# ericbill21/map-dit

Hardware: AMD Instinct MI355X
Metric: latent-images/sec training step, DiT-B/2 bf16 @256 (higher is better)
Workload: dtype bf16; 1 GPU; DiT-B/2 full training step on 32x32x4 latents (fresh batch+fwd+loss+bwd+grad reduction+Adam+2xEMA), all magnitude-preserving features on, bf16 GEMM operands / fp32 accumulate, master and residual fp32; global_batch=256, per_gpu_batch=256, parallelism=dp1, grad_comm=allreduce-fp32-per-stage-overlapped

## Files before the change

include/mapdit.h:

```cpp
#ifndef MAPDIT_H
#define MAPDIT_H

#include <stddef.h>
#include <stdint.h>

#ifdef __cplusplus
extern "C" {
#endif

#define MAPDIT_OK 0
#define MAPDIT_ERR_ARG 1
#define MAPDIT_ERR_HIP 2

const char* mapdit_last_error(void);
int mapdit_abi_version(void);

enum { MAPDIT_NT = 0, MAPDIT_NN = 1, MAPDIT_TN = 2 };

enum {
    MAPDIT_EPI_STORE_BF16 = 0,
    MAPDIT_EPI_STORE_F32 = 1,
    MAPDIT_EPI_SILU2 = 2,
    MAPDIT_EPI_RESID = 3,
    MAPDIT_EPI_DSILU = 4,
    MAPDIT_EPI_SILU2_COND = 5,
    MAPDIT_EPI_SILU2_GRAD = 7,
    MAPDIT_EPI_MUL_AUX = 8,
    MAPDIT_EPI_RMB = 9,
    MAPDIT_EPI_QKV_HEADS = 6,
    MAPDIT_EPI_QKV_HEADS_RAW = 10
};

typedef struct {
    int kind;
    void* out;
    int ldo;
    void* out2;
    const void* aux;
    const float* gate;
    int ldg;
    int rows_per_sample;
    float alpha, beta;
    int accumulate;
    void* out3;
    const float* shift2;
    const float* scale2;
    const float* gain2;
    int ld2;
    int split_k;
    long slab_stride;
    void* out4;
    const void* rmb;
    int rot2;
} mapdit_epilogue_t;

int mapdit_gemm_bf16(int layout, int M, int N, int K, const uint16_t* A, int lda, const uint16_t* B, int ldb,
                     const mapdit_epilogue_t* epi, void* stream);
typedef struct {
    const uint16_t* A; int lda;
    const uint16_t* B; int ldb;
    int M, N;
    float* out; int ldo;
    float alpha;
    long slab_stride;
} mapdit_gemm_group_item_t;
int mapdit_gemm_group_tn_bf16(int n, const mapdit_gemm_group_item_t* items, int K, int split_k, void* stream);
int mapdit_gemm_tile_size(int M, int N);
int mapdit_gemm_tile_size_ex(int M, int N, int split_k_launch);
int mapdit_gemm_tile_size_k(int M, int N, int K, int split_k_launch);
void mapdit_gemm_tuning(int tile, int phases, long band);

enum { MAPDIT_WN_PLAIN = 2 };
int mapdit_weightnorm_fwd(float* W, int rows, int cols, int forced, float out_scale, uint16_t* w_bf16, float* w_f32,
                          float* inv, void* stream);
typedef struct {
    float* W;
    int rows, cols;
    float out_scale;
    int first_block;
    uint16_t* w_bf16;
    float* w_f32;
    uint16_t* w_split3;
    int flags;
} mapdit_wn_job_t;
int mapdit_weightnorm_fwd_batch(const mapdit_wn_job_t* jobs_dev, int njobs, int total_blocks, int forced, void* stream);
int mapdit_weightnorm_bwd(const float* W, float* G, int ldg, int nslabs, long slab_stride, float* dW, int rows,
                          int cols, float out_scale, int accumulate, void* stream);
int mapdit_weightnorm_bwd_batch(const mapdit_wn_job_t* jobs_dev, int njobs, int total_blocks, void* stream);
typedef struct {
    const float* W; float* G; int ldg; int nslabs; long slab_stride; float* dW; int rows, cols; float out_scale; int flags;
} mapdit_wn_bwd_item_t;
int mapdit_weightnorm_bwd_group(int n, const mapdit_wn_bwd_item_t* items, void* stream);
int mapdit_weightnorm_bwd_slim(const float* W, float* G, int ldg, int nslabs, long slab_stride, float* dW, int rows,
                               int cols, float out_scale, int accumulate, void* stream);

typedef struct {
    long lo, hi, first_block;
} mapdit_range_t;

int mapdit_adam_ema_step(float* params, const float* grads, float* exp_avg, float* exp_avg_sq, float* ema_a,
                         float* ema_b, long n, const float* hyper, float beta1, float beta2, float eps, void* stream);
typedef struct {
    float step_size;
    float inv_sqrt_bc2;
    float ema_beta_a, ema_beta_b;
    float grad_scale;
} mapdit_adam_scalars_t;
int mapdit_adam_ema_step_scalars(float* params, const float* grads, float* exp_avg, float* exp_avg_sq, float* ema_a,
                                 float* ema_b, long n, const mapdit_adam_scalars_t* hyper, float beta1, float beta2,
                                 float eps, void* stream);
int mapdit_grad_nonfinite_check(const float* grads, long n, int* status, int step, void* stream);
int mapdit_adam_ema_step_guarded(float* params, const float* grads, float* exp_avg, float* exp_avg_sq, float* ema_a, float* ema_b,
                                 long n, const mapdit_adam_scalars_t* hyper, float beta1, float beta2, float eps,
                                 const int* status, int step, void* stream);
int mapdit_adam_ema_step_ranges(float* params, const float* grads, float* exp_avg, float* exp_avg_sq, float* ema_a, float* ema_b,
                                const mapdit_range_t* ranges_dev, int nranges, long total_blocks, const mapdit_adam_scalars_t* hyper,
                                float beta1, float beta2, float eps, const int* status, int step, void* stream);
int mapdit_grad_nonfinite_check_ranges(const float* grads, const mapdit_range_t* ranges_dev, int nranges, long total_blocks, int* status,
                                       int step, void* stream);

int mapdit_modulate_fwd(const float* x, const float* shift, const float* scale, int ldmod, const float* gain,
                        uint16_t* out, int n_samples, int T, int D, void* stream);

// ... 255 lines not shown
```

map-dit_amd/_lib.py:

```python
from __future__ import annotations

import ctypes as C
import os
import subprocess
import threading

_HERE = os.path.dirname(os.path.abspath(__file__))
LIB_PATH = os.environ.get("MAPDIT_LIB") or os.path.join(_HERE, "libmapdit_hip.so")
CSRC = os.path.join(_HERE, "csrc")

vp, ci, cf, cl = C.c_void_p, C.c_int, C.c_float, C.c_long


class MapditError(RuntimeError):
    pass


class Epilogue(C.Structure):
    _fields_ = [("kind", ci), ("out", vp), ("ldo", ci), ("out2", vp), ("aux", vp), ("gate", vp), ("ldg", ci),
                ("rows_per_sample", ci), ("alpha", cf), ("beta", cf), ("accumulate", ci), ("out3", vp), ("shift2", vp), ("scale2", vp),
                ("gain2", vp), ("ld2", ci), ("split_k", ci), ("slab_stride", cl), ("out4", vp), ("rmb", vp), ("rot2", ci)]


class ResidModBwd(C.Structure):
# ... 95 lines not shown
    "mapdit_fourier_fwd": [vp, vp, vp, vp, ci, ci, vp],
    "mapdit_cond_combine_fwd": [vp, vp, vp, vp, vp, vp, ci, ci, ci, vp],
    "mapdit_cond_combine_bwd": [vp, vp, vp, vp, vp, vp, ci, ci, ci, vp],
    "mapdit_device_error_poll": [vp],
    "mapdit_comm_unique_id": [vp],
    "mapdit_comm_create": [vp, ci, ci, C.POINTER(vp)],
    "mapdit_allreduce_bucket": [vp, vp, cl, vp],
    "mapdit_reduce_scatter_bucket": [vp, vp, cl, vp],
    "mapdit_allgather_bucket": [vp, vp, cl, vp],
    "mapdit_final_out_fwd": [vp, ci, vp, vp, vp, vp, vp, ci, ci, ci, ci, vp],
    "mapdit_final_out_bwd": [vp, vp, ci, vp, vp, vp, vp, vp, ci, vp, vp, vp, vp, cf, ci, ci, ci, ci, vp],
    "mapdit_cfg_combine": [vp, vp, ci, ci, ci, cf, vp],
    "mapdit_q_sample": [vp, vp, vp, vp, ci, vp, ci, ci, vp],
    "mapdit_loss_fwd": [vp, vp, vp, vp, vp, vp, ci, vp, vp, vp, vp, ci, ci, vp],
    "mapdit_loss_bwd": [vp, vp, vp, vp, vp, ci, ci, vp],
    "mapdit_psample_step": [vp, vp, vp, vp, vp, ci, ci, vp, vp, ci, ci, vp],
    "mapdit_ddim_step": [vp, vp, vp, vp, vp, vp, ci, ci, cf, ci, vp, vp, ci, ci, vp],
    "mapdit_obj_loss_fwd": [vp, vp, vp, vp, vp, vp, vp, ci, ci, ci, ci, vp, vp, vp, vp, ci, ci, vp],
    "mapdit_obj_loss_bwd": [vp, vp, vp, vp, vp, ci, ci, ci, vp],
    "mapdit_obj_step": [vp, vp, vp, vp, vp, vp, ci, ci, ci, ci, ci, cf, vp, vp, ci, ci, vp],
    "mapdit_obj_vb_terms": [vp, vp, vp, vp, vp, vp, vp, ci, ci, ci, ci, vp, vp, vp, vp, ci, ci, ci, ci, vp],
    "mapdit_prior_bpd": [vp, vp, vp, ci, vp, vp, vp, ci, ci, vp],
    "mapdit_engine_create": [C.POINTER(Config), ci, vp, C.c_size_t, vp, C.POINTER(vp)],
    "mapdit_engine_bind": [vp, C.POINTER(vp), C.POINTER(vp)],
    "mapdit_engine_prepare_weights": [vp, ci, vp],
    "mapdit_engine_forward": [vp, vp, vp, vp, ci, ci, vp, vp],
    "mapdit_engine_backward": [vp, vp, vp],
    "mapdit_engine_backward_stages": [vp, vp, ci, ci, vp],
    "mapdit_engine_set_shard": [vp, ci, ci],
    "mapdit_engine_set_block_fences": [vp, C.POINTER(vp), ci],
    "mapdit_engine_weight_image": [vp, ci, C.POINTER(vp), C.POINTER(vp), C.POINTER(ci), C.POINTER(ci), C.POINTER(ci)],
    "mapdit_engine_jacobian_shard": [vp, vp],
    "mapdit_engine_set_loss_scale": [vp, cf],
    "mapdit_engine_loss_scale": [vp, C.POINTER(cf)],
    "mapdit_engine_profile_begin": [vp, ci, ci],
    "mapdit_engine_profile_begin_strided": [vp, ci, ci, ci],
    "mapdit_engine_profile_end": [vp, C.POINTER(ci), C.POINTER(C.c_double)],
    "mapdit_engine_peek": [vp, ci, ci, C.POINTER(vp), C.POINTER(C.c_long), C.POINTER(ci), C.POINTER(ci)],
}
for _n in ("weightnorm_fwd", "weightnorm_fwd_batch", "modulate_fwd", "resid_mod_bwd", "rot_modulate_fwd", "qkv_split",
           "qkv_merge_bwd", "attn_cos_fwd", "attn_cos_fwd_rawqk", "attn_cos_fwd_rawqk_save", "qk_cos_normalize", "attn_cos_bwd", "attn_cos_bwd_fused", "attn_sdpa_fwd", "heads_merge_bwd", "ln_modulate_fwd", "ln_bwd_merge", "qkv_split_generic", "qkv_merge_bwd_generic",
           "attn_generic_fwd", "attn_generic_bwd", "patch_embed_fwd", "cond_combine_fwd", "cond_combine_bwd", "final_out_bwd"):
    _SIGS[f"mapdit_{_n}_f16"] = _SIGS[f"mapdit_{_n}"]
for _b, _h in (("gemm_bf16", "gemm_f16"), ("gemm_group_tn_bf16", "gemm_group_tn_f16"), ("f32_to_bf16", "f32_to_f16"), ("f32_to_bf16_2d", "f32_to_f16_2d"),
               ("mpsilu_to_bf16", "mpsilu_to_f16")):
    _SIGS[f"mapdit_{_h}"] = _SIGS[f"mapdit_{_b}"]
_OTHER = {
    "mapdit_last_error": (C.c_char_p, []),
    "mapdit_abi_version": (ci, []),
    "mapdit_gemm_tile_size": (ci, [ci, ci]),
    "mapdit_gemm_tile_size_ex": (ci, [ci, ci, ci]),
    "mapdit_gemm_tile_size_k": (ci, [ci, ci, ci, ci]),
    "mapdit_gemm_tuning": (None, [ci, ci, cl]),
    "mapdit_engine_workspace_bytes": (C.c_size_t, [C.POINTER(Config), ci]),
    "mapdit_engine_destroy": (None, [vp]),
    "mapdit_comm_destroy": (None, [vp]),
}
EXPORTS = sorted(list(_SIGS) + list(_OTHER))

_lock = threading.Lock()
_handle = None


def _source_digest() -> str:
    import hashlib
    h = hashlib.sha256()
    inc = os.path.join(os.path.dirname(_HERE), "include", "mapdit.h")
    files = sorted(os.path.join(CSRC, f) for f in os.listdir(CSRC) if f.endswith((".hip", ".h")) or f == "Makefile") + [inc]
    for f in files:
        h.update(os.path.basename(f).encode() + b"\0")
        with open(f, "rb") as fh:
            h.update(fh.read())
    return h.hexdigest()


def build(force: bool = False) -> str:
    stamp = LIB_PATH + ".src-sha256"
    digest = _source_digest()
    if not force and os.path.exists(LIB_PATH) and os.path.exists(stamp) and open(stamp).read().strip() == digest:
        return LIB_PATH
    if force:
        subprocess.check_call(["make", "-C", CSRC, "clean"])
    subprocess.check_call(["make", "-C", CSRC, "-j8"])
    with open(stamp, "w") as f:
        f.write(digest + "\n")
    return LIB_PATH


class _Lib:
    def __init__(self, cdll):
        self._cdll = cdll
        for name, argtypes in _SIGS.items():
            fn = getattr(cdll, name)
            fn.argtypes = argtypes
            fn.restype = ci
            setattr(self, name[len("mapdit_"):], self._wrap(name, fn))
        for name, (res, argtypes) in _OTHER.items():
            fn = getattr(cdll, name)
            fn.argtypes = argtypes
            fn.restype = res
            setattr(self, name[len("mapdit_"):], fn)

    def _wrap(self, name, fn):
        def call(*args):
            rc = fn(*args)
            if rc != 0:
# ... 25 lines not shown
```

map-dit_amd/csrc/gemm.hip:

```cpp
#include <stdarg.h>
#include <type_traits>
#include <stdio.h>

#include "common.h"

MD_NS_OPEN

constexpr int BM = 128, BN = 128, BKT = 64;
constexpr int TILE_BYTES = 16384;
constexpr int BUF_BYTES = 2 * TILE_BYTES;
constexpr int CS_LD = 132;
constexpr int SMEM_BYTES = BM * CS_LD * 4;

enum { OP_ROW = 0, OP_KMAJ = 1 };

struct GemmP {
    const bf16_t* A;
    const bf16_t* B;
    int lda, ldb;
    int M, N, K;
    int tiles_n;
    int tiles;
    int split_k;
    int band;
// ... 607 lines not shown
#pragma unroll
        for (int ks = 0; ks < 2; ++ks) {
            bf16x8_t fa[4], fb[2];
#pragma unroll
            for (int i = 0; i < 4; ++i) fa[i] = read_frag<OP_ROW>(cur, i * 16, ks, lane);
#pragma unroll
            for (int j = 0; j < 2; ++j) fb[j] = read_frag<BK>(cur + TILE_BYTES, wave * 32 + j * 16, ks, lane);
            if (BK == OP_KMAJ) {
                asm volatile("s_waitcnt lgkmcnt(0)" ::: "memory");
                __builtin_amdgcn_sched_barrier(0);
            }
#pragma unroll
            for (int i = 0; i < 4; ++i)
#pragma unroll
                for (int j = 0; j < 2; ++j) acc[i][j] = MFMA16(fb[j], fa[i], acc[i][j]);
        }
    }
    __syncthreads();
    float* cs = (float*)smem;
#pragma unroll
    for (int i = 0; i < 4; ++i)
#pragma unroll
        for (int j = 0; j < 2; ++j) {
            const int m = i * 16 + (lane & 15);
            const int n = wave * 32 + j * 16 + 4 * (lane >> 4);
            *(f32x4_t*)(cs + m * CS_LD + n) = acc[i][j];
        }
    __syncthreads();
#pragma unroll
    for (int it = 0; it < 4; ++it) {
        const int row = (tid >> 4) + 16 * it, col = (tid & 15) * 8;
        const int gm = m0 + row, gn = n0 + col;
        if (gm < p.M && gn < p.N) {
            float v[8];
            *(f32x4_t*)(v) = *(const f32x4_t*)(cs + row * CS_LD + col);
            *(f32x4_t*)(v + 4) = *(const f32x4_t*)(cs + row * CS_LD + col + 4);
            epi(gm, gn + p.n_off, v, 0);
        }
    }
}

constexpr int BM2 = 256, BN2 = 256;
constexpr int SLOT_BYTES = 16384, KBUF_BYTES = 4 * SLOT_BYTES;
constexpr int OFF_A0 = 0, OFF_A1 = SLOT_BYTES, OFF_B0 = 2 * SLOT_BYTES, OFF_B1 = 3 * SLOT_BYTES;
constexpr int CS2_LD = 260;
constexpr int SMEM2_BYTES = 128 * CS2_LD * 4;
#ifdef MAPDIT_GEMM_STAMPS
constexpr int STAMP_TILES = 12, STAMP_POINTS = 11;
__device__ long long* g_stamps = nullptr;
__device__ long long* g_wg_times = nullptr;
extern "C" __global__ void mapdit_debug_set_wg_times_kernel(long long* p) { g_wg_times = p; }
__device__ int g_stamp_block = -1;
extern "C" __global__ void mapdit_debug_set_stamps_kernel(long long* p, int block) { g_stamps = p; g_stamp_block = block; }
#define G256_STAMP(PT)                                                                              \
    if (stamp_on && t < STAMP_TILES) {                                                              \
        __builtin_amdgcn_sched_barrier(0);                                                          \
        stamp_lds[(wm * STAMP_TILES + t) * STAMP_POINTS + (PT)] = (long long)__builtin_readcyclecounter(); \
        __builtin_amdgcn_sched_barrier(0);                                                          \
    }
#define G256_TSTAMP(IDX)                                                                            \
    if (wave == 0 && (IDX) < 3) {                        \
        __builtin_amdgcn_sched_barrier(0);                                                          \
        kl_[(IDX) % 3] = (long long)__builtin_readcyclecounter();                                       \
        __builtin_amdgcn_sched_barrier(0);                                                          \
    }                                                                                               \
    if (stamp_on && wave == 0) {                                                                    \
        __builtin_amdgcn_sched_barrier(0);                                                          \
        stamp_lds[2 * STAMP_TILES * STAMP_POINTS + (IDX)] = (long long)__builtin_readcyclecounter(); \
        __builtin_amdgcn_sched_barrier(0);                                                          \
    }
#define G256_RSTAMP(IDX)                                                                            \
    if (stamp_on && wave == 0) {                                                                    \
        __builtin_amdgcn_sched_barrier(0);                                                          \
        stamp_lds[2 * STAMP_TILES * STAMP_POINTS + (IDX)] = (long long)__builtin_amdgcn_s_memrealtime(); \
        __builtin_amdgcn_sched_barrier(0);                                                          \
    }
#define G256_STAMPS_OUT()                                                                           \
    if (g_wg_times && wave == 0 && lane == 0) {                                                     \
        long long* r_ = g_wg_times + 4 * (long long)bid;                                     \
        r_[0] = wg_r0; r_[1] = (long long)__builtin_amdgcn_s_memrealtime();                         \
        const long long now_ = (long long)__builtin_readcyclecounter();                             \
        r_[2] = now_ - wg_t0;                                                                       \
                       \
        r_[3] = ((long long)__builtin_amdgcn_s_getreg(((4 - 1) << 11) | (0 << 6) | 20) & 0xff) |    \
                (((kl_[2] - kl_[1]) & 0xffffff) << 8) | (((kl_[1] - wg_t0) & 0xffff) << 32) |       \
                (((now_ - kl_[2]) & 0xffff) << 48);                                                 \
    }                                                                                               \
    if (stamp_on) {                                                                                 \
        for (int i = 0; i < STAMP_TILES * STAMP_POINTS; ++i)                                        \
            g_stamps[wm * STAMP_TILES * STAMP_POINTS + i] = stamp_lds[wm * STAMP_TILES * STAMP_POINTS + i]; \
        if (wave == 0)                                                                              \
            for (int i = 0; i < 8; ++i) g_stamps[2 * STAMP_TILES * STAMP_POINTS + i] = stamp_lds[2 * STAMP_TILES * STAMP_POINTS + i]; \
    }
#else
#define G256_STAMP(PT)
#define G256_TSTAMP(IDX)
#define G256_RSTAMP(IDX)
#define G256_STAMPS_OUT()
#endif

template <int SIDE> __device__ __forceinline__ int half_map(int i, int h) {
    return SIDE == 0 ? ((i >> 6) * 128 + h * 64 + (i & 63)) : ((i >> 5) * 64 + h * 32 + (i & 31));
}

template <int KIND, int SIDE, bool KTAIL>
__device__ __forceinline__ void stage_half(const bf16_t* __restrict__ G, int ld, int idx0, int idx_max, int k0, int kmax, int h,
// ... 435 lines not shown
    __shared__ __attribute__((aligned(16))) char smem[kReduce<Epi> ? SMEM2_BYTES + 3 * 8 * 256 * 4 : SMEM2_BYTES];
#endif
    const int total = p.tiles * p.split_k;
    stagger_start(p);
    for (int v = blockIdx.x; v < total; v += gridDim.x) {
        gemm256_tile<AK, BK, Epi, KTAIL, FE>(p, epi, smem, v, total);
        __syncthreads();
    }
}

constexpr int GROUP_MAX = 4;
struct GroupArgs {
    GemmP p[GROUP_MAX];
    EpiStoreF32 e[GROUP_MAX];
    int first[GROUP_MAX + 1];
    int n;
};
__global__ __launch_bounds__(512, 2) void gemm_mfma256_group_kernel(GroupArgs g) {
#ifdef MAPDIT_GEMM_STAMPS
    __shared__ __attribute__((aligned(16))) char smem[SMEM2_BYTES + (2 * STAMP_TILES * STAMP_POINTS + 8) * 8];
#else
    __shared__ __attribute__((aligned(16))) char smem[SMEM2_BYTES];
#endif
    const int total = g.first[g.n];
    for (int v = blockIdx.x; v < total; v += gridDim.x) {
        int i = 0;
        while (i + 1 < g.n && v >= g.first[i + 1]) ++i;
        gemm256_tile<OP_KMAJ, OP_KMAJ, EpiStoreF32, false, false>(g.p[i], g.e[i], smem, v - g.first[i], g.first[i + 1] - g.first[i]);
        __syncthreads();
    }
}

struct TileCoord { int m0, n0, z, tile, kbeg, nk; };
__device__ __forceinline__ TileCoord tile_coord(const GemmP& p, const int bid, const int nwg) {
    const int xcd = bid & 7, q = nwg >> 3, r = nwg & 7;
    const int wg = (xcd < r ? xcd * (q + 1) : r * (q + 1) + (xcd - r) * q) + (bid >> 3);
    TileCoord c;
    c.z = wg / p.tiles;
    c.tile = wg - c.z * p.tiles;
    const int tiles_m = p.tiles / p.tiles_n;
    const int bsz = tiles_m * p.band;
    const int bidx = c.tile / bsz, rem = c.tile - bidx * bsz;
    const int bw = (bidx + 1) * p.band <= p.tiles_n ? p.band : p.tiles_n - bidx * p.band;
    c.m0 = (rem / bw) * BM2;
    c.n0 = (bidx * p.band + rem % bw) * BN2;
    const int nkt = (p.K + BKT - 1) / BKT, kbase = nkt / p.split_k, krem = nkt % p.split_k;
    c.kbeg = (c.z * kbase + (c.z < krem ? c.z : krem)) * BKT;
    c.nk = kbase + (c.z < krem ? 1 : 0);
    return c;
}

constexpr int WPRIV_BYTES = 4096;
constexpr int SMEM_W_BYTES = 2 * KBUF_BYTES + 8 * WPRIV_BYTES;

template <int AK, int BK, bool KTAIL>
__device__ __forceinline__ void g256_prologue(const GemmP& p, const TileCoord& c, char* smem, int wave, int lane) {
    stage_half<AK, 0, KTAIL>(p.A, p.lda, c.m0, p.M, c.kbeg, p.K, 0, smem + OFF_A0, wave, lane);
    stage_half<BK, 1, KTAIL>(p.B, p.ldb, c.n0, p.N, c.kbeg, p.K, 0, smem + OFF_B0, wave, lane);
    stage_half<BK, 1, KTAIL>(p.B, p.ldb, c.n0, p.N, c.kbeg, p.K, 1, smem + OFF_B1, wave, lane);
    stage_half<AK, 0, KTAIL>(p.A, p.lda, c.m0, p.M, c.kbeg, p.K, 1, smem + OFF_A1, wave, lane);
    if (c.nk > 1) {
        char* b1 = smem + KBUF_BYTES;
        stage_half<AK, 0, KTAIL>(p.A, p.lda, c.m0, p.M, c.kbeg + BKT, p.K, 0, b1 + OFF_A0, wave, lane);
        stage_half<BK, 1, KTAIL>(p.B, p.ldb, c.n0, p.N, c.kbeg + BKT, p.K, 0, b1 + OFF_B0, wave, lane);
        stage_half<BK, 1, KTAIL>(p.B, p.ldb, c.n0, p.N, c.kbeg + BKT, p.K, 1, b1 + OFF_B1, wave, lane);
    }
}

#ifndef MAPDIT_EPI_PD_AUX
#define MAPDIT_EPI_PD_AUX 2
#endif
template <class Epi> constexpr bool kWaveEpilogue = true;
template <class Epi> constexpr bool kWaveEpilogueAnyK = true;
template <> constexpr bool kWaveEpilogue<EpiResid> = false;
template <> constexpr bool kWaveEpilogue<EpiStoreF32> = false;
template <> constexpr bool kWaveEpilogueAnyK<EpiStoreBf16> = false;
template <class Epi> constexpr int kEpiPrefetch = 2;
template <class Epi> constexpr bool kEpiPipeline = true;
template <> constexpr int kEpiPrefetch<EpiResid> = 1;
template <> constexpr int kEpiPrefetch<EpiMulAux> = MAPDIT_EPI_PD_AUX;
template <> constexpr int kEpiPrefetch<EpiDSilu> = MAPDIT_EPI_PD_AUX;
template <> constexpr bool kEpiPipeline<EpiResid> = false;
template <class Epi, bool INTERIOR>
__device__ __forceinline__ void g256w_epilogue(const GemmP& p, const Epi& epi, const TileCoord& c, f32x4_t (&acc)[8][4],
                                               char* priv, const int wave, const int lane) {
    const int wm = wave >> 2, wn = wave & 3;
    const int cch = lane & 7, rsub = lane >> 3;
    const int wrow = lane & 15, wq = lane >> 4;
    const int gn = c.n0 + wn * 64 + cch * 8;
    const bool col_ok = INTERIOR || gn < p.N;
    typename Epi::Tile tctx;
    if (col_ok) tctx = epi.tile_begin(c.m0, (c.m0 + BM2 <= p.M ? c.m0 + BM2 : p.M) - 1, gn);
    f32x4_t* b = (f32x4_t*)priv;
    constexpr int PD = kEpiPrefetch<Epi>;
    constexpr bool PIPE = kEpiPipeline<Epi>;
    typename Epi::Aux aux[8][2];
    const int mw = c.m0 + wm * 128 + rsub;
    auto row_of = [&](int r, int s) { return mw + (r >> 2) * 64 + (r & 3) * 16 + 8 * s; };
    int woff[4], roff[2][2];
#pragma unroll
    for (int j = 0; j < 4; ++j) woff[j] = wrow * 16 + ((4 * j + wq) ^ (wrow & 7));
#pragma unroll
    for (int s = 0; s < 2; ++s) {
        const int rr = rsub + 8 * s;
        roff[s][0] = rr * 16 + ((2 * cch) ^ (rr & 7));
        roff[s][1] = rr * 16 + ((2 * cch + 1) ^ (rr & 7));
    }
#pragma unroll
    for (int r = 0; r < PD; ++r)
#pragma unroll
        for (int s = 0; s < 2; ++s)
            if (INTERIOR || (row_of(r, s) < p.M && col_ok)) aux[r][s] = epi.load(row_of(r, s), gn);
    f32x4_t cur[2][2], nxt[2][2];
    if (PIPE) {
#pragma unroll
        for (int j = 0; j < 4; ++j) b[woff[j]] = acc[0][j];
#pragma unroll
        for (int s = 0; s < 2; ++s) { cur[s][0] = b[roff[s][0]]; cur[s][1] = b[roff[s][1]]; }
    }
#pragma unroll
    for (int r = 0; r < 8; ++r) {
        if (r + PD < 8) {
#pragma unroll
            for (int s = 0; s < 2; ++s)
                if (INTERIOR || (row_of(r + PD, s) < p.M && col_ok)) aux[r + PD][s] = epi.load(row_of(r + PD, s), gn);
        }
        if (PIPE && r + 1 < 8) {
#pragma unroll
            for (int j = 0; j < 4; ++j) b[woff[j]] = acc[r + 1][j];
#pragma unroll
            for (int s = 0; s < 2; ++s) { nxt[s][0] = b[roff[s][0]]; nxt[s][1] = b[roff[s][1]]; }
        }
        if (!PIPE) {
#pragma unroll
            for (int j = 0; j < 4; ++j) b[woff[j]] = acc[r][j];
#pragma unroll
            for (int s = 0; s < 2; ++s) { cur[s][0] = b[roff[s][0]]; cur[s][1] = b[roff[s][1]]; }
        }
#pragma unroll
        for (int s = 0; s < 2; ++s) {
            float v[8];
            *(f32x4_t*)(v) = cur[s][0];
            *(f32x4_t*)(v + 4) = cur[s][1];
            if (INTERIOR || (row_of(r, s) < p.M && col_ok)) epi.apply(row_of(r, s), gn, v, c.z, aux[r][s], tctx);
        }
        if (PIPE) {
#pragma unroll
            for (int s = 0; s < 2; ++s) { cur[s][0] = nxt[s][0]; cur[s][1] = nxt[s][1]; }
        }
    }
}

template <int AK, int BK, class Epi, bool KTAIL = false>
__global__ __launch_bounds__(512, 2) void gemm_mfma256w_kernel(GemmP p, Epi epi) {
    __shared__ __attribute__((aligned(16))) char smem[SMEM_W_BYTES];
    const int total = p.tiles * p.split_k;
    int v = blockIdx.x;
    if (v >= total) return;
    stagger_start(p);
    constexpr bool TR_ASM2 = AK == OP_KMAJ;
    TileCoord c = tile_coord(p, v, total);
    {
        const int tid0 = threadIdx.x;
        g256_prologue<AK, BK, KTAIL>(p, c, smem, __builtin_amdgcn_readfirstlane(tid0 >> 6), tid0 & 63);
    }
    bool first = true;
#ifdef MAPDIT_GEMM_STAMPS
    long long ph_[4] = {0, 0, 0, 0};
    int ph_tiles_ = 0;
#define GW_STAMP(VAR) __builtin_amdgcn_sched_barrier(0); const long long VAR = (long long)__builtin_readcyclecounter(); __builtin_amdgcn_sched_barrier(0)
#else
#define GW_STAMP(VAR)
#endif
    for (;;) {
        int tid_ = threadIdx.x;
        asm volatile("" : "+v"(tid_));
        const int tid = tid_, lane = tid & 63;
        const int wave = __builtin_amdgcn_readfirstlane(tid >> 6);
        const int wm = wave >> 2, wn = wave & 3;
        const int m0 = c.m0, n0 = c.n0, kbeg = c.kbeg, nk = c.nk;
        f32x4_t acc[8][4];
#pragma unroll
        for (int i = 0; i < 8; ++i)
#pragma unroll
            for (int j = 0; j < 4; ++j) acc[i][j] = f32x4_t{0.f, 0.f, 0.f, 0.f};
        bf16x8_t fa[4][2], fb0[2][2], fb1[2][2];
        auto load_a = [&](const char* slot) {
#pragma unroll
            for (int i = 0; i < 4; ++i)
#pragma unroll
                for (int ks = 0; ks < 2; ++ks) fa[i][ks] = read_frag<AK, TR_ASM2>(slot, wm * 64 + i * 16, ks, lane);
        };
        GW_STAMP(ts0_);
        if (first && nk > 1) asm volatile("s_waitcnt vmcnt(8)" ::: "memory");
        else asm volatile("s_waitcnt vmcnt(0)" ::: "memory");
        __builtin_amdgcn_sched_barrier(0);
        __builtin_amdgcn_s_barrier();
        __builtin_amdgcn_sched_barrier(0);
        if (wm == 1) {
            __builtin_amdgcn_s_barrier();
            __builtin_amdgcn_sched_barrier(0);
        }
        GW_STAMP(ts1_);
        for (int t = 0; t < nk; ++t) {
            char* cur = smem + (t & 1) * KBUF_BYTES;
            char* nxt = smem + ((t + 1) & 1) * KBUF_BYTES;
            const int k1 = kbeg + (t + 1) * BKT, k2 = kbeg + (t + 2) * BKT;
            const bool has1 = t + 1 < nk, has2 = t + 2 < nk;
            load_a(cur + OFF_A0);
            G256_LOAD_B(fb0, cur + OFF_B0);
            G256_LOAD_B(fb1, cur + OFF_B1);
            if (has1) {
                stage_half<AK, 0, KTAIL>(p.A, p.lda, m0, p.M, k1, p.K, 1, nxt + OFF_A1, wave, lane);
                asm volatile("s_waitcnt vmcnt(8)" ::: "memory");
            } else {
                asm volatile("s_waitcnt vmcnt(0)" ::: "memory");
            }
            G256_END_LOAD();
            G256_MFMA(0, 0, fb0);
            G256_MFMA(0, 1, fb1);
            G256_END_MFMA();
            load_a(cur + OFF_A1);
            if (has2) {
                stage_half<AK, 0, KTAIL>(p.A, p.lda, m0, p.M, k2, p.K, 0, cur + OFF_A0, wave, lane);
                stage_half<BK, 1, KTAIL>(p.B, p.ldb, n0, p.N, k2, p.K, 0, cur + OFF_B0, wave, lane);
                stage_half<BK, 1, KTAIL>(p.B, p.ldb, n0, p.N, k2, p.K, 1, cur + OFF_B1, wave, lane);
                asm volatile("s_waitcnt vmcnt(8)" ::: "memory");
            } else if (has1) {
                asm volatile("s_waitcnt vmcnt(2)" ::: "memory");
            } else {
                asm volatile("s_waitcnt vmcnt(0)" ::: "memory");
            }
            G256_END_LOAD();
            G256_MFMA(1, 1, fb1);
            G256_MFMA(1, 0, fb0);
            G256_END_MFMA();
        }
        if (wm == 0) {
            __builtin_amdgcn_s_barrier();
            __builtin_amdgcn_sched_barrier(0);
        }
        GW_STAMP(ts2_);
        const int vn = v + (int)gridDim.x;
        TileCoord cn = c;
        if (vn < total) {
            cn = tile_coord(p, vn, total);
            g256_prologue<AK, BK, KTAIL>(p, cn, smem, wave, lane);
        }
        GW_STAMP(ts3_);
        if (c.m0 + BM2 <= p.M && c.n0 + BN2 <= p.N)
            g256w_epilogue<Epi, true>(p, epi, c, acc, smem + 2 * KBUF_BYTES + wave * WPRIV_BYTES, wave, lane);
        else
            g256w_epilogue<Epi, false>(p, epi, c, acc, smem + 2 * KBUF_BYTES + wave * WPRIV_BYTES, wave, lane);
#ifdef MAPDIT_GEMM_STAMPS
        {
            GW_STAMP(ts4_);
            ph_[0] += ts1_ - ts0_; ph_[1] += ts2_ - ts1_; ph_[2] += ts3_ - ts2_; ph_[3] += ts4_ - ts3_;
            ++ph_tiles_;
            if ((vn >= total) && g_wg_times && (wave & 3) == 0 && lane == 0) {
                long long* r_ = g_wg_times + 16 * (long long)blockIdx.x + 8 * (wave >> 2);
                r_[0] = ph_[0]; r_[1] = ph_[1]; r_[2] = ph_[2]; r_[3] = ph_[3]; r_[4] = ph_tiles_;
            }
        }
#endif
        if (vn >= total) break;
        v = vn;
        c = cn;
        first = false;
    }
}

template <class Epi>
__global__ void gemm_simple_kernel(const bf16_t* __restrict__ A, long sam, long sak, const bf16_t* __restrict__ B,
                                   long sbn, long sbk, int M, int N, int K, Epi epi) {
    const int chunks = N >> 3;
    const long id = (long)blockIdx.x * blockDim.x + threadIdx.x;
    if (id >= (long)M * chunks) return;
    const int m = (int)(id / chunks), n = (int)(id % chunks) * 8;
    float v[8] = {0, 0, 0, 0, 0, 0, 0, 0};
    for (int k = 0; k < K; ++k) {
        const float a = up16(A[m * sam + k * sak]);
#pragma unroll
        for (int i = 0; i < 8; ++i) v[i] += a * up16(B[(n + i) * sbn + k * sbk]);
    }
    epi(m, n, v);
}

MD_NS_CLOSE

#ifdef MAPDIT_GEMM_STAMPS
extern "C" void mapdit_debug_set_stamps(long long* p) {
    hipLaunchKernelGGL(mapdit_debug_set_stamps_kernel, dim3(1), dim3(1), 0, 0, p, -1);
    (void)hipDeviceSynchronize();
}
extern "C" void mapdit_debug_set_wg_times(long long* p) {
    hipLaunchKernelGGL(mapdit_debug_set_wg_times_kernel, dim3(1), dim3(1), 0, 0, p);
    (void)hipDeviceSynchronize();
}
extern "C" void mapdit_debug_set_stamps_block(long long* p, int block) {
    hipLaunchKernelGGL(mapdit_debug_set_stamps_kernel, dim3(1), dim3(1), 0, 0, p, block);
    (void)hipDeviceSynchronize();
}
#endif

static int gemm_phases_arg(int v) { return v == 4 || v == 6 || v == 7 ? v : 2; }

struct GemmEnv {
    int tile = 0;
    int phases = 2;
    long band = 0;
    int old_tile_rule = 0;
    int persist = 256;
    int keep_mask = 1;
    int nsplit = 1;
    int fast_epi = 1;
    int band768 = 3;
    int stagger = -1;
    GemmEnv() {
        if (const char* e = getenv("MAPDIT_GEMM_PERSIST")) persist = atoi(e);
        if (const char* e = getenv("MAPDIT_KEEP")) keep_mask = atoi(e);
        if (const char* e = getenv("MAPDIT_GEMM_NSPLIT")) nsplit = atoi(e);
        if (const char* e = getenv("MAPDIT_GEMM_STAGGER")) stagger = atoi(e);
        if (const char* e = getenv("MAPDIT_GEMM_BAND768")) band768 = atoi(e) > 0 ? atoi(e) : 3;
        if (const char* e = getenv("MAPDIT_GEMM_FE")) fast_epi = atoi(e);
        if (const char* e = getenv("MAPDIT_GEMM_TILE_RULE")) old_tile_rule = e[0] == 'o';
        if (const char* e = getenv("MAPDIT_GEMM_TILE")) tile = atoi(e);
        if (const char* e = getenv("MAPDIT_GEMM_PHASES")) phases = gemm_phases_arg(atoi(e));
        if (const char* e = getenv("MAPDIT_GEMM_BAND")) band = atol(e);
    }
};
GemmEnv& mapdit_gemm_env_ref();
static GemmEnv& gemm_env() { return mapdit_gemm_env_ref(); }
#if MAPDIT_DT == 0
GemmEnv& mapdit_gemm_env_ref() {
    static GemmEnv env;
    return env;
}
extern "C" void mapdit_gemm_tuning(int tile, int phases, long band) {
    GemmEnv& e = gemm_env();
    e.tile = tile;
    e.phases = gemm_phases_arg(phases);
    e.band = band;
}

extern "C" int mapdit_gemm_tile_size_k(int M, int N, int K, int split_k_launch) {
    const int force = gemm_env().tile;
    if (force == 128 || force == 256) return force;
    if (!(M >= 512 && N >= 256)) return 128;
    const long t256 = (long)cdiv(M, 256) * cdiv(N, 256);
    if (split_k_launch) {
        if (t256 < 12) return 128;
        if (!gemm_env().old_tile_rule && (double)M * N < 0.85 * (double)t256 * 65536.0) return 128;
        if (K > 0 && !gemm_env().old_tile_rule) {
            const long slabs = 256 / t256 > 0 ? 256 / t256 : 1;
            if ((K / 64) / slabs < 24) return 128;
        }
        return 256;
    }
    if (t256 < 128) return 128;
    if (!gemm_env().old_tile_rule && t256 > 256 && t256 <= 320) return 128;
    return 256;
}
extern "C" int mapdit_gemm_tile_size_ex(int M, int N, int split_k_launch) { return mapdit_gemm_tile_size_k(M, N, 0, split_k_launch); }
extern "C" int mapdit_gemm_tile_size(int M, int N) { return mapdit_gemm_tile_size_ex(M, N, 0); }
#endif

MD_NS_OPEN

template <class Epi> constexpr bool kHasTail = false;
template <> constexpr bool kHasTail<EpiStoreF32> = true;

template <class F>
inline void with_operand_kinds(int layout, F&& f) {
    using Row = std::integral_constant<int, OP_ROW>;
    using Kmaj = std::integral_constant<int, OP_KMAJ>;
    if (layout == MAPDIT_NT) f(Row(), Row());
    else if (layout == MAPDIT_NN) f(Row(), Kmaj());
    else f(Kmaj(), Kmaj());
}

template <class Epi>
int launch(int layout, int M, int N, int K, const bf16_t* A, int lda, const bf16_t* B, int ldb, Epi epi,
           hipStream_t st, int split_k = 1, int n_off = 0, bool force128 = false) {
    bool a_kmaj = false, b_kmaj = false;
    with_operand_kinds(layout, [&](auto ak, auto bk) { a_kmaj = ak.value == OP_KMAJ; b_kmaj = bk.value == OP_KMAJ; });
    if constexpr (!kReduce<Epi>) {
        if (!force128 && n_off == 0 && split_k == 1 && gemm_env().nsplit && N % 256 == 128 && N >= 384 && K % BKT == 0 &&
            gemm_env().tile != 128 && M >= 512 && (long)cdiv(M, 256) * ((N - 128) / 256) >= 192 &&
            (long)cdiv(M, 256) * ((N - 128) / 256) <= 256 && !(((uintptr_t)A | (uintptr_t)B) & 15) &&
            lda % 8 == 0 && ldb % 8 == 0 && !(a_kmaj && M % 8 != 0)) {
            const int N1 = N - 128;
            const bf16_t* B2 = b_kmaj ? B + N1 : B + (size_t)N1 * ldb;
            if (!(((uintptr_t)B2) & 15)) {
                const int rc = launch(layout, M, N1, K, A, lda, B, ldb, epi, st, 1, 0, false);
                if (rc != MAPDIT_OK) return rc;
                return launch(layout, M, 128, K, A, lda, B2, ldb, epi, st, 1, N1, true);
            }
        }
    }
    const bool ktail = K % BKT != 0;
    bool mfma = (K % 8 == 0) && (N % 8 == 0) && K > 0 && (!ktail || kHasTail<Epi>);
    if (a_kmaj && (M % 8 != 0 || lda % 8 != 0)) mfma = false;
    if (b_kmaj && (ldb % 8 != 0)) mfma = false;
    if (!a_kmaj && lda % 8 != 0) mfma = false;
    if (!b_kmaj && ldb % 8 != 0) mfma = false;
    if (((uintptr_t)A | (uintptr_t)B) & 15) mfma = false;
    if constexpr (kReduce<Epi>) {
        if (!mfma || ktail || mapdit_gemm_tile_size_k(M, N, K, 0) != 256) {
            mapdit_set_error("gemm: this epilogue needs the 256x256 MFMA path (M=%d N=%d K=%d: K %% 64 == 0, M >= 512, N >= 256, aligned operands)", M, N, K);
            return MAPDIT_ERR_ARG;
        }
    }
    if (split_k > 1 && (!mfma || split_k > (K + BKT - 1) / BKT)) {
        mapdit_set_error("gemm: split_k=%d needs the MFMA path and split_k <= ceil(K/64) (K=%d)", split_k, K);
        return MAPDIT_ERR_ARG;
    }
    if (mfma && !force128 && mapdit_gemm_tile_size_k(M, N, K, split_k > 1) == 256) {
        GemmP p{A, B, lda, ldb, M, N, K, cdiv(N, BN2), 0, split_k, 0, 2, 0, 0};
        p.tiles = cdiv(M, BM2) * p.tiles_n;
        p.phases = gemm_env().phases;
        const bool be = gemm_env().band > 0;
        long band = be ? gemm_env().band : (long)(2.5 * 1024 * 1024) / ((long)BN2 * (K / split_k) * 2);
        if (!be && band < 4) band = p.tiles_n;
        if (!be && layout == MAPDIT_NT && split_k == 1 && K <= 768 && p.tiles_n >= 6 && p.tiles_n % gemm_env().band768 == 0) band = gemm_env().band768;
        if (band < 1 || band > p.tiles_n) band = p.tiles_n;
        p.band = (int)band;
        int grid = p.tiles * split_k;
        if (gemm_env().persist && grid >= 3 * gemm_env().persist) {
            grid = gemm_env().persist;
            const int sg = gemm_env().stagger;
            p.stagger = sg >= 0 ? sg : (std::is_same<Epi, EpiResid>::value ? 2 : 0);
        }
        bool use_w = false;
        if constexpr (!kReduce<Epi>)
            use_w = p.phases == 6 || (p.phases == 2 && kWaveEpilogue<Epi> && (kWaveEpilogueAnyK<Epi> || K / split_k <= 1024));
        if (p.phases == 7 || p.phases == 6) p.phases = 2;
        bool fe = false;
        if constexpr (kFastEpi<Epi>)
            fe = gemm_env().fast_epi && M % BM2 == 0 && N % BN2 == 0 && epi.fast_ok();
        auto go = [&](auto tail) {
            constexpr bool TAIL = decltype(tail)::value;
            with_operand_kinds(layout, [&](auto ak, auto bk) {
                if constexpr (!kReduce<Epi>) {
                    if (use_w) { hipLaunchKernelGGL((gemm_mfma256w_kernel<ak.value, bk.value, Epi, TAIL>), dim3(grid), dim3(512), 0, st, p, epi); return; }
                }
                if constexpr (kFastEpi<Epi> && !TAIL) {
                    if (fe) { hipLaunchKernelGGL((gemm_mfma256_kernel<ak.value, bk.value, Epi, false, true>), dim3(grid), dim3(512), 0, st, p, epi); return; }
                }
                hipLaunchKernelGGL((gemm_mfma256_kernel<ak.value, bk.value, Epi, TAIL>), dim3(grid), dim3(512), 0, st, p, epi);
            });
        };
        if constexpr (kHasTail<Epi>) {
            if (ktail) {
                go(std::true_type());
                MD_LAUNCH_CHECK();
                return MAPDIT_OK;
            }
        }
        go(std::false_type());
    } else if (mfma) {
        if constexpr (std::is_same<Epi, EpiResid>::value || std::is_same<Epi, EpiStoreBf16>::value) {
            static const bool t64_env = [] { const char* v = getenv("MAPDIT_GEMM_TILE64"); return !(v && v[0] == '0'); }();
            const long t128 = (long)cdiv(M, BM) * cdiv(N, BN);
            if (t64_env && !a_kmaj && !ktail && split_k == 1 && t128 <= 160 && M >= 256) {
                GemmP p{A, B, lda, ldb, M, N, K, cdiv(N, BN), 0, 1, 0, 4, n_off, 0};
                p.tiles = cdiv(M, 64) * p.tiles_n;
                with_operand_kinds(layout, [&](auto, auto bk) {
                    hipLaunchKernelGGL((gemm_mfma64_kernel<bk.value, Epi>), dim3(p.tiles), dim3(256), 0, st, p, epi);
                });
                MD_LAUNCH_CHECK();
                return MAPDIT_OK;
            }
        }
        GemmP p{A, B, lda, ldb, M, N, K, cdiv(N, BN), 0, split_k, 0, 4, n_off, 0};
        p.tiles = cdiv(M, BM) * p.tiles_n;
        const int grid = p.tiles * split_k;
        if constexpr (kHasTail<Epi>) {
            if (ktail) {
                with_operand_kinds(layout, [&](auto ak, auto bk) {
                    hipLaunchKernelGGL((gemm_mfma_kernel<ak.value, bk.value, Epi, true>), dim3(grid), dim3(256), 0, st, p, epi);
                });
// ... 153 lines not shown
```

Baseline: 5960 latent-img/s.

## Prefetch next persistent tile's K-slices during current tile's tail and epilogue

In the persistent 256x256 wave-epilogue GEMM kernel, the loader now looks up to two tiles ahead. During the last K iterations and before the epilogue it stages the first K-slices of the next tile into the double buffer, instead of running a full prologue after the epilogue. Buffer parity is carried across tiles, and barrier placement is reworked so waves skip the per-tile entry sync. This is meant to hide global-load latency at tile boundaries. The cost is more complex waitcnt and barrier logic, with some risk of hazards. It also adds a persist-rounds knob and debug stamp hooks.

```diff
diff --git a/include/mapdit.h b/include/mapdit.h
--- a/include/mapdit.h
+++ b/include/mapdit.h
@@ -69,6 +69,7 @@
 int mapdit_gemm_tile_size_ex(int M, int N, int split_k_launch);
 int mapdit_gemm_tile_size_k(int M, int N, int K, int split_k_launch);
 void mapdit_gemm_tuning(int tile, int phases, long band);
+void mapdit_gemm_persist(int workgroups, int min_rounds);
 
 enum { MAPDIT_WN_PLAIN = 2 };
 int mapdit_weightnorm_fwd(float* W, int rows, int cols, int forced, float out_scale, uint16_t* w_bf16, float* w_f32,
diff --git a/map-dit_amd/_lib.py b/map-dit_amd/_lib.py
--- a/map-dit_amd/_lib.py
+++ b/map-dit_amd/_lib.py
@@ -171,6 +171,7 @@
     "mapdit_gemm_tile_size_ex": (ci, [ci, ci, ci]),
     "mapdit_gemm_tile_size_k": (ci, [ci, ci, ci, ci]),
     "mapdit_gemm_tuning": (None, [ci, ci, cl]),
+    "mapdit_gemm_persist": (None, [ci, ci]),
     "mapdit_engine_workspace_bytes": (C.c_size_t, [C.POINTER(Config), ci]),
     "mapdit_engine_destroy": (None, [vp]),
     "mapdit_comm_destroy": (None, [vp]),
diff --git a/map-dit_amd/csrc/gemm.hip b/map-dit_amd/csrc/gemm.hip
--- a/map-dit_amd/csrc/gemm.hip
+++ b/map-dit_amd/csrc/gemm.hip
@@ -683,6 +683,10 @@
 extern "C" __global__ void mapdit_debug_set_wg_times_kernel(long long* p) { g_wg_times = p; }
 __device__ int g_stamp_block = -1;
 extern "C" __global__ void mapdit_debug_set_stamps_kernel(long long* p, int block) { g_stamps = p; g_stamp_block = block; }
+constexpr int WST_TILES = 12, WST_KT = 12, WST_REC = 64;
+__device__ long long* g_wstamps = nullptr;
+__device__ int g_wstamp_block = -1;
+extern "C" __global__ void mapdit_debug_set_wstamps_kernel(long long* p, int block) { g_wstamps = p; g_wstamp_block = block; }
 #define G256_STAMP(PT)                                                                              \
     if (stamp_on && t < STAMP_TILES) {                                                              \
         __builtin_amdgcn_sched_barrier(0);                                                          \
@@ -1224,20 +1228,6 @@
 
 constexpr int WPRIV_BYTES = 4096;
 constexpr int SMEM_W_BYTES = 2 * KBUF_BYTES + 8 * WPRIV_BYTES;
-
-template <int AK, int BK, bool KTAIL>
-__device__ __forceinline__ void g256_prologue(const GemmP& p, const TileCoord& c, char* smem, int wave, int lane) {
-    stage_half<AK, 0, KTAIL>(p.A, p.lda, c.m0, p.M, c.kbeg, p.K, 0, smem + OFF_A0, wave, lane);
-    stage_half<BK, 1, KTAIL>(p.B, p.ldb, c.n0, p.N, c.kbeg, p.K, 0, smem + OFF_B0, wave, lane);
-    stage_half<BK, 1, KTAIL>(p.B, p.ldb, c.n0, p.N, c.kbeg, p.K, 1, smem + OFF_B1, wave, lane);
-    stage_half<AK, 0, KTAIL>(p.A, p.lda, c.m0, p.M, c.kbeg, p.K, 1, smem + OFF_A1, wave, lane);
-    if (c.nk > 1) {
-        char* b1 = smem + KBUF_BYTES;
-        stage_half<AK, 0, KTAIL>(p.A, p.lda, c.m0, p.M, c.kbeg + BKT, p.K, 0, b1 + OFF_A0, wave, lane);
-        stage_half<BK, 1, KTAIL>(p.B, p.ldb, c.n0, p.N, c.kbeg + BKT, p.K, 0, b1 + OFF_B0, wave, lane);
-        stage_half<BK, 1, KTAIL>(p.B, p.ldb, c.n0, p.N, c.kbeg + BKT, p.K, 1, b1 + OFF_B1, wave, lane);
-    }
-}
 
 #ifndef MAPDIT_EPI_PD_AUX
 #define MAPDIT_EPI_PD_AUX 2
@@ -1323,26 +1313,70 @@
     }
 }
 
+struct KTileAhead { int m0, n0, k; bool ok; };
+
 template <int AK, int BK, class Epi, bool KTAIL = false>
 __global__ __launch_bounds__(512, 2) void gemm_mfma256w_kernel(GemmP p, Epi epi) {
     __shared__ __attribute__((aligned(16))) char smem[SMEM_W_BYTES];
     const int total = p.tiles * p.split_k;
-    int v = blockIdx.x;
-    if (v >= total) return;
+    if ((int)blockIdx.x >= total) return;
     stagger_start(p);
     constexpr bool TR_ASM2 = AK == OP_KMAJ;
-    TileCoord c = tile_coord(p, v, total);
+    const int stride = (int)gridDim.x;
+    int v = blockIdx.x;
+    auto coord_at = [&](int vv) {
+        TileCoord r{0, 0, 0, 0, 0, 0};
+        if (vv < total) r = tile_coord(p, vv, total);
+        return r;
+    };
+    TileCoord c = tile_coord(p, v, total), c1 = coord_at(v + stride), c2 = coord_at(v + 2 * stride);
+    auto ahead = [&](int u) {
+        const bool in1 = u < c1.nk;
+        const TileCoord& s = in1 ? c1 : c2;
+        return KTileAhead{s.m0, s.n0, s.kbeg + (in1 ? u : 0) * BKT, c1.nk > 0 && s.nk > 0};
+    };
     {
         const int tid0 = threadIdx.x;
-        g256_prologue<AK, BK, KTAIL>(p, c, smem, __builtin_amdgcn_readfirstlane(tid0 >> 6), tid0 & 63);
+        const int wave = __builtin_amdgcn_readfirstlane(tid0 >> 6), lane = tid0 & 63;
+        stage_half<AK, 0, KTAIL>(p.A, p.lda, c.m0, p.M, c.kbeg, p.K, 0, smem + OFF_A0, wave, lane);
+        stage_half<BK, 1, KTAIL>(p.B, p.ldb, c.n0, p.N, c.kbeg, p.K, 0, smem + OFF_B0, wave, lane);
+        stage_half<BK, 1, KTAIL>(p.B, p.ldb, c.n0, p.N, c.kbeg, p.K, 1, smem + OFF_B1, wave, lane);
+        stage_half<AK, 0, KTAIL>(p.A, p.lda, c.m0, p.M, c.kbeg, p.K, 1, smem + OFF_A1, wave, lane);
+        const KTileAhead a = c.nk > 1 ? KTileAhead{c.m0, c.n0, c.kbeg + BKT, true} : ahead(0);
+        if (a.ok) {
+            char* b1 = smem + KBUF_BYTES;
+            stage_half<AK, 0, KTAIL>(p.A, p.lda, a.m0, p.M, a.k, p.K, 0, b1 + OFF_A0, wave, lane);
+            stage_half<BK, 1, KTAIL>(p.B, p.ldb, a.n0, p.N, a.k, p.K, 0, b1 + OFF_B0, wave, lane);
+            stage_half<BK, 1, KTAIL>(p.B, p.ldb, a.n0, p.N, a.k, p.K, 1, b1 + OFF_B1, wave, lane);
+            asm volatile("s_waitcnt vmcnt(8)" ::: "memory");
+        } else {
+            asm volatile("s_waitcnt vmcnt(0)" ::: "memory");
+        }
+        __builtin_amdgcn_sched_barrier(0);
+        __builtin_amdgcn_s_barrier();
+        __builtin_amdgcn_sched_barrier(0);
+        if (wave >> 2 == 1) {
+            __builtin_amdgcn_s_barrier();
+            __builtin_amdgcn_sched_barrier(0);
+        }
     }
     bool first = true;
+    int par = 0;
 #ifdef MAPDIT_GEMM_STAMPS
     long long ph_[4] = {0, 0, 0, 0};
     int ph_tiles_ = 0;
 #define GW_STAMP(VAR) __builtin_amdgcn_sched_barrier(0); const long long VAR = (long long)__builtin_readcyclecounter(); __builtin_amdgcn_sched_barrier(0)
+    const bool wst_wg_ = g_wstamps && (int)blockIdx.x == g_wstamp_block;
+#define GW_KSTAMP(PT)                                                                                             \
+    if (wst_wg_ && (wave & 3) == 0 && lane == 0 && t < WST_KT) {                                                  \
+        __builtin_amdgcn_sched_barrier(0);                                                                        \
+        ((long long*)(smem + 2 * KBUF_BYTES + wave * WPRIV_BYTES))[t * 4 + (PT)] = (long long)__builtin_readcyclecounter(); \
+        __builtin_amdgcn_sched_barrier(0);                                                                        \
+    }
+    long long ts_prev_ = (long long)__builtin_readcyclecounter();
 #else
 #define GW_STAMP(VAR)
+#define GW_KSTAMP(PT)
 #endif
     for (;;) {
         int tid_ = threadIdx.x;
@@ -1363,81 +1397,113 @@
 #pragma unroll
                 for (int ks = 0; ks < 2; ++ks) fa[i][ks] = read_frag<AK, TR_ASM2>(slot, wm * 64 + i * 16, ks, lane);
         };
-        GW_STAMP(ts0_);
-        if (first && nk > 1) asm volatile("s_waitcnt vmcnt(8)" ::: "memory");
-        else asm volatile("s_waitcnt vmcnt(0)" ::: "memory");
-        __builtin_amdgcn_sched_barrier(0);
-        __builtin_amdgcn_s_barrier();
-        __builtin_amdgcn_sched_barrier(0);
-        if (wm == 1) {
-            __builtin_amdgcn_s_barrier();
-            __builtin_amdgcn_sched_barrier(0);
-        }
+#ifdef MAPDIT_GEMM_STAMPS
+        const long long ts0_ = ts_prev_;
+#endif
         GW_STAMP(ts1_);
         for (int t = 0; t < nk; ++t) {
-            char* cur = smem + (t & 1) * KBUF_BYTES;
-            char* nxt = smem + ((t + 1) & 1) * KBUF_BYTES;
+            char* cur = smem + ((par + t) & 1) * KBUF_BYTES;
+            char* nxt = smem + ((par + t + 1) & 1) * KBUF_BYTES;
             const int k1 = kbeg + (t + 1) * BKT, k2 = kbeg + (t + 2) * BKT;
             const bool has1 = t + 1 < nk, has2 = t + 2 < nk;
+            const bool head = !first && t == 0;
+            GW_KSTAMP(0);
             load_a(cur + OFF_A0);
             G256_LOAD_B(fb0, cur + OFF_B0);
             G256_LOAD_B(fb1, cur + OFF_B1);
-            if (has1) {
+            if (head) {
+            } else if (has1) {
                 stage_half<AK, 0, KTAIL>(p.A, p.lda, m0, p.M, k1, p.K, 1, nxt + OFF_A1, wave, lane);
                 asm volatile("s_waitcnt vmcnt(8)" ::: "memory");
             } else {
-                asm volatile("s_waitcnt vmcnt(0)" ::: "memory");
+                const KTileAhead a = ahead(0);
+                if (a.ok) {
+                    stage_half<AK, 0, KTAIL>(p.A, p.lda, a.m0, p.M, a.k, p.K, 1, nxt + OFF_A1, wave, lane);
+                    asm volatile("s_waitcnt vmcnt(8)" ::: "memory");
+                } else {
+                    asm volatile("s_waitcnt vmcnt(0)" ::: "memory");
+                }
             }
             G256_END_LOAD();
+            GW_KSTAMP(1);
             G256_MFMA(0, 0, fb0);
             G256_MFMA(0, 1, fb1);
             G256_END_MFMA();
+            GW_KSTAMP(2);
             load_a(cur + OFF_A1);
             if (has2) {
                 stage_half<AK, 0, KTAIL>(p.A, p.lda, m0, p.M, k2, p.K, 0, cur + OFF_A0, wave, lane);
                 stage_half<BK, 1, KTAIL>(p.B, p.ldb, n0, p.N, k2, p.K, 0, cur + OFF_B0, wave, lane);
                 stage_half<BK, 1, KTAIL>(p.B, p.ldb, n0, p.N, k2, p.K, 1, cur + OFF_B1, wave, lane);
-                asm volatile("s_waitcnt vmcnt(8)" ::: "memory");
-            } else if (has1) {
-                asm volatile("s_waitcnt vmcnt(2)" ::: "memory");
+                if (head) asm volatile("s_waitcnt vmcnt(6)" ::: "memory");
+                else asm volatile("s_waitcnt vmcnt(8)" ::: "memory");
             } else {
-                asm volatile("s_waitcnt vmcnt(0)" ::: "memory");
+                const KTileAhead a = ahead(t + 2 - nk);
+                if (a.ok) {
+                    stage_half<AK, 0, KTAIL>(p.A, p.lda, a.m0, p.M, a.k, p.K, 0, cur + OFF_A0, wave, lane);
+                    stage_half<BK, 1, KTAIL>(p.B, p.ldb, a.n0, p.N, a.k, p.K, 0, cur + OFF_B0, wave, lane);
+                    stage_half<BK, 1, KTAIL>(p.B, p.ldb, a.n0, p.N, a.k, p.K, 1, cur + OFF_B1, wave, lane);
+                    if (head) asm volatile("s_waitcnt vmcnt(6)" ::: "memory");
+                    else asm volatile("s_waitcnt vmcnt(8)" ::: "memory");
+                } else if (!head && (has1 || c1.nk > 0)) {
+                    asm volatile("s_waitcnt vmcnt(2)" ::: "memory");
+                } else {
+                    asm volatile("s_waitcnt vmcnt(0)" ::: "memory");
+                }
             }
             G256_END_LOAD();
+            GW_KSTAMP(3);
             G256_MFMA(1, 1, fb1);
             G256_MFMA(1, 0, fb0);
-            G256_END_MFMA();
-        }
-        if (wm == 0) {
-            __builtin_amdgcn_s_barrier();
-            __builtin_amdgcn_sched_barrier(0);
+            if (has1 || wm == 0) { G256_END_MFMA(); }
         }
         GW_STAMP(ts2_);
-        const int vn = v + (int)gridDim.x;
-        TileCoord cn = c;
-        if (vn < total) {
-            cn = tile_coord(p, vn, total);
-            g256_prologue<AK, BK, KTAIL>(p, cn, smem, wave, lane);
-        }
+        {
+            const KTileAhead a = ahead(1);
+            if (a.ok) {
+                stage_half<AK, 0, KTAIL>(p.A, p.lda, a.m0, p.M, a.k, p.K, 1, smem + ((par + nk - 1) & 1) * KBUF_BYTES + OFF_A1, wave, lane);
+                asm volatile("s_waitcnt vmcnt(8)" ::: "memory");
+            } else if (c1.nk > 0) {
+                asm volatile("s_waitcnt vmcnt(0)" ::: "memory");
+            }
+        }
+        const TileCoord c3 = coord_at(v + 3 * stride);
         GW_STAMP(ts3_);
+#ifdef MAPDIT_GEMM_STAMPS
+        if (wst_wg_ && (wave & 3) == 0 && ph_tiles_ < WST_TILES && lane < 4 * WST_KT)
+            g_wstamps[((wave >> 2) * WST_TILES + ph_tiles_) * WST_REC + lane] = ((const long long*)(smem + 2 * KBUF_BYTES + wave * WPRIV_BYTES))[lane];
+#endif
         if (c.m0 + BM2 <= p.M && c.n0 + BN2 <= p.N)
             g256w_epilogue<Epi, true>(p, epi, c, acc, smem + 2 * KBUF_BYTES + wave * WPRIV_BYTES, wave, lane);
         else
             g256w_epilogue<Epi, false>(p, epi, c, acc, smem + 2 * KBUF_BYTES + wave * WPRIV_BYTES, wave, lane);
+        const bool last = c1.nk == 0;
 #ifdef MAPDIT_GEMM_STAMPS
         {
             GW_STAMP(ts4_);
             ph_[0] += ts1_ - ts0_; ph_[1] += ts2_ - ts1_; ph_[2] += ts3_ - ts2_; ph_[3] += ts4_ - ts3_;
+            if (wst_wg_ && (wave & 3) == 0 && ph_tiles_ < WST_TILES && lane == 0) {
+                long long* r_ = g_wstamps + ((wave >> 2) * WST_TILES + ph_tiles_) * WST_REC + WST_REC - 16;
+                r_[0] = ts0_; r_[1] = ts1_; r_[2] = ts2_; r_[3] = ts3_; r_[4] = ts4_;
+            }
+            ts_prev_ = ts4_;
             ++ph_tiles_;
-            if ((vn >= total) && g_wg_times && (wave & 3) == 0 && lane == 0) {
+            if (last && g_wg_times && (wave & 3) == 0 && lane == 0) {
                 long long* r_ = g_wg_times + 16 * (long long)blockIdx.x + 8 * (wave >> 2);
                 r_[0] = ph_[0]; r_[1] = ph_[1]; r_[2] = ph_[2]; r_[3] = ph_[3]; r_[4] = ph_tiles_;
             }
         }
 #endif
-        if (vn >= total) break;
-        v = vn;
-        c = cn;
+        if (wm == 1) { G256_END_MFMA(); }
+        if (last) {
+            if (wm == 0) { G256_END_MFMA(); }
+            break;
+        }
+        par = (par + nk) & 1;
+        v += stride;
+        c = c1;
+        c1 = c2;
+        c2 = c3;
         first = false;
     }
 }
@@ -1469,6 +1535,10 @@
     hipLaunchKernelGGL(mapdit_debug_set_wg_times_kernel, dim3(1), dim3(1), 0, 0, p);
     (void)hipDeviceSynchronize();
 }
+extern "C" void mapdit_debug_set_wstamps(long long* p, int block) {
+    hipLaunchKernelGGL(mapdit_debug_set_wstamps_kernel, dim3(1), dim3(1), 0, 0, p, block);
+    (void)hipDeviceSynchronize();
+}
 extern "C" void mapdit_debug_set_stamps_block(long long* p, int block) {
     hipLaunchKernelGGL(mapdit_debug_set_stamps_kernel, dim3(1), dim3(1), 0, 0, p, block);
     (void)hipDeviceSynchronize();
@@ -1483,6 +1553,7 @@
     long band = 0;
     int old_tile_rule = 0;
     int persist = 256;
+    int persist_rounds = 3;
     int keep_mask = 1;
     int nsplit = 1;
     int fast_epi = 1;
@@ -1515,6 +1586,12 @@
     e.band = band;
 }
 
+extern "C" void mapdit_gemm_persist(int workgroups, int min_rounds) {
+    GemmEnv& e = gemm_env();
+    e.persist = workgroups > 0 ? workgroups : 0;
+    e.persist_rounds = min_rounds > 0 ? min_rounds : 3;
+}
+
 extern "C" int mapdit_gemm_tile_size_k(int M, int N, int K, int split_k_launch) {
     const int force = gemm_env().tile;
     if (force == 128 || force == 256) return force;
@@ -1598,7 +1675,7 @@
         if (band < 1 || band > p.tiles_n) band = p.tiles_n;
         p.band = (int)band;
         int grid = p.tiles * split_k;
-        if (gemm_env().persist && grid >= 3 * gemm_env().persist) {
+        if (gemm_env().persist && grid >= gemm_env().persist_rounds * gemm_env().persist) {
             grid = gemm_env().persist;
             const int sg = gemm_env().stagger;
             p.stagger = sg >= 0 ? sg : (std::is_same<Epi, EpiResid>::value ? 2 : 0);
```

New measurement: 6008 latent-img/s, median of 6. Within noise of the previous version (+0.8%).
